# 111116/zdr

Hardware: AMD Instinct MI355X
Metric: Msamples/s fwd+PRB-bwd, cbox 512x512 spp=256 (higher is better)
Workload: dtype f32; 1 GPU; cbox path integrator 512x512 spp=256, forward + PRB backward w.r.t. the 1024x1024x4 material (BASELINE configs[2]); sampler=cmj, accel=brute, rccl_ranks=1, backend=none

## Files before the change

### zdr_amd/csrc/integrators.h

```cpp
#pragma once
#include <type_traits>
#include "accel.h"
#include "internal.h"
#include "microfacet.h"
#include "zdr.h"

ZD float tent_warp1(float u) {
    return (u < 0.5f) ? (fsqrt(2.0f * u) - 1.0f) : (1.0f - fsqrt(2.0f - 2.0f * u));
}

template <int SK, bool PACKED = false>
ZD void pixel_ray(const RenderCfg &R, const SamplerCfg &C, Sampler &smp, int x, int y, f3 &o, f3 &d) {
    f2 off = PACKED ? sampler_pixel_offset<SK>(C, smp) : sampler_next2<SK>(C, smp);
    if (R.use_tent) { off.x = tent_warp1(off.x) + 0.5f; off.y = tent_warp1(off.y) + 0.5f; }
    float px = R.two_over_w * ((float)x + off.x) - 1.0f;
    float py = R.two_over_h * ((float)y + off.y) - 1.0f;
    py *= R.aspect;
    px *= R.cam_tan; py *= R.cam_tan;
    o = ld3(R.cam_o);
    d = normalize((ld3(R.cam_right) * px - ld3(R.cam_upp) * py) + ld3(R.cam_fwd));
}

struct Counters { uint32_t c[8]; };
enum { C_SAMPLES, C_CLOSEST, C_HITS, C_SHADOW, C_SHADED, C_EMIT_BSDF, C_NAN, C_SHADOW_TRACED };
// ... 149 lines not shown
            }
        } else if (ENV && S.env_count > 0) {
            em = env_lookup(S, direction_to_uv(wi));
            pdf_light = env_sampled_light_pdf(S, wi, S.env_count + S.light_count);
            lit = true;
        }
        if (lit && (em.x > 0.0f || em.y > 0.0f || em.z > 0.0f)) {
            GgxTerms g = ggx_terms(wo, wi_local, roughness);
            float pdf_bsdf = ggx_pdf_from(g, wo, wi_local);
            float mis = balanced_heuristic(pdf_bsdf, pdf_light);
            float inv_p = rcp(pdf_bsdf);
            f3 beta = ggx_brdf_from(g, wi_local, diffuse) * inv_p;
            COUNT(C_EMIT_BSDF);
            radiance = radiance + (beta * mis) * em;
            if constexpr (LG) {
                if (h2.slot >= 0) { l_bsdf->w = beta * mis; l_bsdf->light = emit_light_of(S, hit_inst); }
            }
            if (BWD) {
                float dl_; float4 gr = brdf_grad(wi_local.z * ZDR_INV_PI, ggx_dfdr_from(g, wo, wi_local, roughness, dl_), (em * (mis * inv_p)) * le_grad);
                mat_grad.x += gr.x; mat_grad.y += gr.y; mat_grad.z += gr.z; mat_grad.w += gr.w;
            }
        }
        if constexpr (EG) {
            if (h2.slot < 0 && S.env_count > 0) {
                GgxTerms g = ggx_terms(wo, wi_local, roughness);
                float pdf_bsdf = ggx_pdf_from(g, wo, wi_local);
                e_bsdf->w = (ggx_brdf_from(g, wi_local, diffuse) * rcp(pdf_bsdf)) * balanced_heuristic(pdf_bsdf, pdf_light);
                e_bsdf->uv = direction_to_uv(wi);
            }
        }
    }
    if (BWD) { grad = mat_grad; guv = it.uv; }
    return radiance;
}

struct PathVertex {
    f2 uv;
    f3 bW;  float cL, dfLdr;
    f3 neeM;
    f3 bpq; float c, dfdr;
    f3 T, fLW;
    float dlnp;
    int rr;
    f3 bnorm;
};

struct PathState {
    f3 o, d, beta, L;
    float pdf_bsdf;
    int depth;
    Sampler smp;
};

template <bool BWD, bool STATS, bool ENV, bool MT = false>
ZD bool path_arrive(const DScene &S, PathState &ps, const Hit &h, Interaction &it, f3 &term_Li, Counters &cnt, float *term_plfrac = nullptr,
                    const int32_t *inst_slot = nullptr, EnvTerm *env_hit = nullptr, EmitTerm *emit_hit = nullptr) {
    if (h.slot < 0) {
        if (ENV && S.env_count > 0) {
            const f2 euv = direction_to_uv(ps.d);
            f3 em = env_lookup(S, euv);
            float pdf_light = env_sampled_light_pdf(S, ps.d, S.env_count + S.light_count);
            float mis = balanced_heuristic(ps.pdf_bsdf, pdf_light);
            if (env_hit) { env_hit->w = ps.beta * mis; env_hit->uv = euv; }
            ps.L = ps.L + (ps.beta * mis) * em;
            if (BWD) { term_Li = em * mis;
                       if (term_plfrac) *term_plfrac = (ps.pdf_bsdf + pdf_light > 1e-4f) ? pdf_light * rcp(ps.pdf_bsdf + pdf_light) : 0.0f; }
        }
        return true;
    }
    COUNT(C_HITS);
    it = surface_interact(S, h);
    if (dot(-ps.d, it.ng) < 1e-4f || dot(-ps.d, it.ns) < 1e-4f) return true;
    f3 em = xyz(S.emission4[it.inst]);
    if (em.x > 0.0f || em.y > 0.0f || em.z > 0.0f) {
        float pdf_light = sample_light_pdf<ENV>(S, ps.o, it.inst, h.slot, it.p);
        float mis = balanced_heuristic(ps.pdf_bsdf, pdf_light);
        if (emit_hit) { emit_hit->w = ps.beta * mis; emit_hit->light = emit_light_of(S, it.inst); }
        ps.L = ps.L + (ps.beta * mis) * em;
        if (BWD) { term_Li = em * mis;
                   if (term_plfrac) *term_plfrac = (ps.pdf_bsdf + pdf_light > 1e-4f) ? pdf_light * rcp(ps.pdf_bsdf + pdf_light) : 0.0f; }
        if (STATS && ps.depth > 0) cnt.c[C_EMIT_BSDF]++;
        return true;
    }
    if constexpr (MT) {
        it.mat = inst_slot[it.inst];
        return it.mat < 0;
    }
    if (it.inst > 0) return true;
    return false;
}

struct ShadeCtx { f3 diffuse; float roughness; Onb onb; f3 wo, wil; LightSample light; float u_lobe; f2 u_dir; uint32_t i_rr; bool pre; };
struct NeeTerms { f3 dL, bW, fLW, neeM; float cL, dfLdr; };

template <int SK, bool BWD, bool STATS, bool ENV, bool MT = false, bool LG = false>
ZD ShadeCtx shade_ctx(const DScene &S, const RenderCfg &R, const SamplerCfg &C, const KernelIO &io, PathState &ps, const Interaction &it, PathVertex &pv, Counters &cnt,
                      f2 *env_uv = nullptr, int *mesh_light = nullptr) {
    ShadeCtx x;
    float4 m;
    if constexpr (MT) m = read_bsdf_in(io.material, io.mt.m[it.mat], it.uv);
    else m = read_bsdf(io.material, it.uv, R.tex_h, R.tex_w);
    x.diffuse = mk3(m.x, m.y, m.z); x.roughness = m.w;
    COUNT(C_SHADED);
    if (BWD) {
        pv.uv = it.uv; pv.bW = mk3(0.0f); pv.cL = 0.0f; pv.dfLdr = 0.0f; pv.bpq = mk3(0.0f); pv.c = 0.0f; pv.dfdr = 0.0f;
        pv.T = mk3(0.0f); pv.fLW = mk3(0.0f); pv.bnorm = mk3(0.0f); pv.neeM = mk3(0.0f); pv.dlnp = 0.0f; pv.rr = 0;
    }
    x.onb = make_onb(it.ns);
    x.wo = to_local(x.onb, -ps.d);
    x.pre = (SK == 0) && !ENV && cmj_can_batch(C);
    x.u_lobe = 0.0f; x.u_dir.x = 0.0f; x.u_dir.y = 0.0f; x.i_rr = 0u;
    if (x.pre) {
        const VertexSamples v = cmj_vertex_samples(C, ps.smp);
        x.u_lobe = v.u_lobe; x.u_dir = v.u_dir; x.i_rr = v.i_rr;
        x.light = sample_light<ENV, LG>(S, it.p, v.u_pick, [&]() { return v.u_prim; }, [&]() { return v.u_pt; }, env_uv, mesh_light);
    } else {
        float u_pick = sampler_next<SK>(C, ps.smp);
        x.light = sample_light<ENV, LG>(S, it.p, u_pick, [&]() { return sampler_next<SK>(C, ps.smp); }, [&]() { return sampler_next2<SK>(C, ps.smp); }, env_uv, mesh_light);
    }
    x.wil = to_local(x.onb, x.light.wi);
    return x;
}

template <bool BWD, bool EG = false>
ZD NeeTerms nee_terms(const ShadeCtx &x, f3 beta_in, f3 *env_w = nullptr) {
    NeeTerms n; n.dL = n.bW = n.fLW = n.neeM = mk3(0.0f); n.cL = 0.0f; n.dfLdr = 0.0f;
    GgxTerms g = ggx_terms(x.wo, x.wil, x.roughness);
    f3 bsdf = ggx_brdf_from(g, x.wil, x.diffuse);
    float pb = ggx_pdf_from(g, x.wo, x.wil);
    float mis = balanced_heuristic(x.light.pdf, pb);
    float inv_dn = rcp(fmaxf(x.light.pdf, 1e-4f));
    n.dL = (((beta_in * bsdf) * mis) * x.light.eval) * inv_dn;
    if constexpr (EG) *env_w = ((beta_in * bsdf) * mis) * inv_dn;
    if (BWD) {
        f3 W = (x.light.eval * mis) * inv_dn;
        float dlnpL;
        n.bW = beta_in * W; n.cL = x.wil.z * ZDR_INV_PI; n.dfLdr = ggx_dfdr_from(g, x.wo, x.wil, x.roughness, dlnpL);
        n.fLW = bsdf * W;
        float pbf = (x.light.pdf + pb > 1e-4f) ? pb * rcp(x.light.pdf + pb) : 0.0f;
        n.neeM = ((beta_in * bsdf) * W) * (pbf * dlnpL);
    }
    return n;
// ... 136 lines not shown
ZD PrimaryQueue queue_init(const KernelIO &io) {
    PrimaryQueue r; r.base = io.ring + (size_t)blockIdx.x * (ZDR_QUEUE_ENTRIES * 2); r.head = 0; r.tail = 0;
    return r;
}
ZD uint32_t lane_rank(unsigned long long mask) {
    return __builtin_amdgcn_mbcnt_hi((unsigned)(mask >> 32), __builtin_amdgcn_mbcnt_lo((unsigned)mask, 0u));
}

struct NoEnvMiss { ZD void operator()(const EnvTerm &) const {} };
struct NoEmitHit { ZD void operator()(const EmitTerm &) const {} };
template <int SK, class A, bool BWD, bool STATS, bool ENV, bool MT = false, class MISS = NoEnvMiss, class EMIT = NoEmitHit>
ZD void primary_refill(const DScene &S, const RenderCfg &R, const SamplerCfg &C, int *lds, int x, int y, bool valid, unsigned long long cam_mask,
                       uint32_t perm_seed, int bank, uint32_t &next_sample, uint32_t s_end, PrimaryQueue &q, f3 &sum, Counters &cnt,
                       const int32_t *inst_slot = nullptr, MISS on_miss = MISS(), EMIT on_emit = EMIT()) {
    constexpr bool EG = !std::is_same<MISS, NoEnvMiss>::value;
    constexpr bool LG = !std::is_same<EMIT, NoEmitHit>::value;
    for (int b = 0; b < ZDR_RING_BATCH && next_sample < s_end; b++, next_sample++) {
        bool park = false;
        float4 e0 = make_float4(0.0f, 0.0f, 0.0f, 0.0f), e1 = e0;
        EnvTerm miss; env_term_clear(miss);
        if (valid) {
            PathState ps;
            ps.smp = sampler_make<SK>(C, (uint32_t)x, (uint32_t)y, perm_seed, next_sample);
            pixel_ray<SK>(R, C, ps.smp, x, y, ps.o, ps.d);
            ps.beta = mk3(1.0f); ps.L = mk3(0.0f); ps.pdf_bsdf = 1e30f; ps.depth = 0;
            COUNT(C_SAMPLES); COUNT(C_CLOSEST);
            Hit h = A::closest_camera(S, lds, ps.o, ps.d, cam_mask);
            Interaction it; f3 tl;
            EmitTerm seen; emit_term_clear(seen);
            const bool ended = path_arrive<false, STATS, ENV, MT>(S, ps, h, it, tl, cnt, nullptr, inst_slot, EG ? &miss : nullptr, LG ? &seen : nullptr);
            if constexpr (LG) on_emit(seen);
            if (ended) {
                if (!BWD) {
                    if (!any_nan(ps.L)) sum = sum + clamp_radiance(ps.L);
                    else COUNT(C_NAN);
                }
            } else {
                park = true;
                e0 = make_float4(ps.d.x, ps.d.y, ps.d.z, h.u);
                e1 = make_float4(h.v, __int_as_float(h.slot), __uint_as_float(ps.smp.state), __uint_as_float(((uint32_t)threadIdx.x << 26) | ((uint32_t)bank << 25) | next_sample));
            }
        }
        if constexpr (EG) on_miss(miss);
        const unsigned long long m = __ballot(park);
        if (park) {
            float4 *e = q.base + (size_t)((q.tail + lane_rank(m)) % ZDR_QUEUE_ENTRIES) * 2;
            e[0] = e0; e[1] = e1;
        }
        q.tail += (uint32_t)__popcll(m);
    }
    __builtin_amdgcn_fence(__ATOMIC_RELEASE, "wavefront");
}

template <int SK, bool MT = false>
ZD int primary_pop(const DScene &S, const SamplerCfg &C, bool idle, const uint32_t *lds_perm, const int *lds_origin,
                   PrimaryQueue &q, PathState &ps, Interaction &it, const int32_t *inst_slot = nullptr) {
    const unsigned long long m = __ballot(idle);
    const uint32_t avail = q.tail - q.head, rank = lane_rank(m), want = (uint32_t)__popcll(m);
    const bool take = idle && rank < avail;
    int pix = -1;
    __builtin_amdgcn_fence(__ATOMIC_ACQUIRE, "wavefront");
    if (take) {
        const float4 *e = q.base + (size_t)((q.head + rank) % ZDR_QUEUE_ENTRIES) * 2;
        float4 a = e[0], b = e[1];
        Hit h; h.slot = __float_as_int(b.y); h.u = a.w; h.v = b.x; h.t = 0.0f;
        it = surface_interact(S, h);
        if constexpr (MT) it.mat = inst_slot[it.inst];
        ps.d = mk3(a.x, a.y, a.z); ps.o = mk3(0.0f);
        ps.beta = mk3(1.0f); ps.L = mk3(0.0f); ps.pdf_bsdf = 1e30f; ps.depth = 0;
        const uint32_t key = __float_as_uint(b.w);
        const int p = (int)(key >> 26), bank = (int)((key >> 25) & 1u);
        pix = bank * 64 + p;
        ps.smp.px = (uint32_t)(lds_origin[bank * 2] + (p & 7)); ps.smp.py = (uint32_t)(lds_origin[bank * 2 + 1] + (p >> 3));
        ps.smp.sample_index = key & 0x01ffffffu;
        ps.smp.dimension = 2;
        ps.smp.permutation_seed = lds_perm ? lds_perm[pix] : ((SK == 0) ? xxhash32_4(ps.smp.px, ps.smp.py, C.seed, 0u) : 0u);
        ps.smp.state = __float_as_uint(b.z);
    }
    q.head += (want < avail) ? want : avail;
    return pix;
}

struct PackedVertex { float4 a, b, c, d, e; };

ZD PackedVertex pack_vertex(const PathVertex &v, f3 g, int mode = ZDR_PRB_EXPECTATION) {
    PackedVertex p;
    p.a = brdf_grad(v.cL, v.dfLdr, v.bW * g);
    if (mode == ZDR_PRB_EXPECTATION) p.a.w -= dot(g, v.neeM);
    f3 Q = v.bpq * v.c;
    float r = (v.c > 0.0f) ? v.dfdr * rcp(v.c) : 0.0f;
    p.b = make_float4(Q.x, Q.y, Q.z, r);
    p.c = make_float4(v.T.x, v.T.y, v.T.z, v.uv.x);
    f3 gA = g * v.fLW;
    p.d = make_float4(gA.x, gA.y, gA.z, v.uv.y);
    f3 e = (v.rr == 2) ? v.bnorm : ((v.rr == 1) ? mk3(-1.0f, 0.0f, 0.0f) : mk3(0.0f));
    p.e = make_float4(e.x, e.y, e.z, v.dlnp);
    if (mode == ZDR_PRB_DETACHED) p.e = make_float4(0.0f, 0.0f, 0.0f, 0.0f);
    if (mode == ZDR_PRB_LITERAL) p.e = make_float4(v.bnorm.x, v.bnorm.y, v.bnorm.z, 0.0f);
    return p;
}

struct SweepState { f3 A, Lv; float s, Z, tw; };

ZD float4 sweep_vertex(const PackedVertex &p, SweepState &S, f2 &uv, int mode = ZDR_PRB_EXPECTATION) {
    const f3 w = mk3(0.212671f, 0.715160f, 0.072169f);
    f3 Aeff = S.A;
    if (mode == ZDR_PRB_LITERAL) {
        Aeff = mk3(p.e.x, p.e.y, p.e.z) * S.Lv;
    } else if (p.e.x < 0.0f) {
        Aeff = S.A + w * S.s; S.s = 0.0f; S.Z = 0.0f;
    } else if (p.e.x + p.e.y + p.e.z > 0.0f) {
        f3 b = mk3(p.e.x, p.e.y, p.e.z);
        float ba = dot(b, S.A);
        Aeff = S.A - w * ba; S.s += ba; S.Z = dot(b, S.Lv);
    }
    f3 ct = mk3(p.b.x, p.b.y, p.b.z) * Aeff;
    float4 g = make_float4(p.a.x + ct.x, p.a.y + ct.y, p.a.z + ct.z,
                           p.a.w + p.b.w * (ct.x + ct.y + ct.z) + p.e.w * (S.Z + S.tw));
    S.tw = 0.0f;
    f3 T = mk3(p.c.x, p.c.y, p.c.z), gA = mk3(p.d.x, p.d.y, p.d.z);
// ... 6 lines not shown
```

### zdr_amd/csrc/zdr_kernels.hip

```cpp
#include <algorithm>
#include <cstddef>
#include <cstdlib>
#include <map>
#include <mutex>
#include <tuple>
#include <type_traits>
#include "integrators.h"
#include "zdr.h"

#define WAVE 64

struct WorkItem { int x, y, pix; bool valid; uint32_t s_begin, s_end; int chunk, tile, tile_local; };

ZD WorkItem decode_item(const RenderCfg &R, int logical) {
    const int nblocks = R.ntiles * R.nchunks;
    WorkItem w;
    w.valid = logical >= 0 && logical < nblocks;
    const int tl = w.valid ? logical / R.nchunks : 0;
    w.chunk = w.valid ? logical - tl * R.nchunks : 0;
    const int number = tl * R.shard_count + R.shard_index;
    const int ty = number / R.tiles_x;
    int tx = number - ty * R.tiles_x + ty * R.shard_skew;
    tx -= (tx / R.tiles_x) * R.tiles_x;
    w.tile = ty * R.tiles_x + tx; w.tile_local = tl;
// ... 111 lines not shown
struct ItemBanks {
    int logical[2];
    uint32_t inflight[2];
};

struct PathKArgs { DScene S; RenderCfg R; SamplerCfg C; KernelIO io; };
#define ZDR_PATH_KERNEL_PARAMS DScene S_, RenderCfg R_, SamplerCfg C_, KernelIO io_
static constexpr size_t zdr_align_up(size_t x, size_t a) { return (x + a - 1) / a * a; }
static_assert(std::is_trivially_copyable<PathKArgs>::value && std::is_standard_layout<PathKArgs>::value, "kernel arguments are copied bytewise");
static_assert(offsetof(PathKArgs, S) == 0, "first kernel argument at offset 0 of the kernarg segment");
static_assert(offsetof(PathKArgs, R) == zdr_align_up(sizeof(DScene), alignof(RenderCfg)), "PathKArgs does not mirror the kernarg packing");
static_assert(offsetof(PathKArgs, C) == zdr_align_up(offsetof(PathKArgs, R) + sizeof(RenderCfg), alignof(SamplerCfg)), "PathKArgs does not mirror the kernarg packing");
static_assert(offsetof(PathKArgs, io) == zdr_align_up(offsetof(PathKArgs, C) + sizeof(SamplerCfg), alignof(KernelIO)), "PathKArgs does not mirror the kernarg packing");
static_assert(alignof(DScene) <= 8 && alignof(RenderCfg) <= 8 && alignof(SamplerCfg) <= 8 && alignof(KernelIO) <= 8, "an over-aligned member would change the kernarg packing");
typedef __attribute__((address_space(4))) const char karg_byte_t;
ZD const PathKArgs &kargs_fresh() {
    karg_byte_t *p = (karg_byte_t *)__builtin_amdgcn_kernarg_segment_ptr();
    asm volatile("" : "+s"(p));
    return *(const PathKArgs *)p;
}
#define ZDR_KARGS_BEGIN const PathKArgs *ka = &kargs_fresh();
#define ZDR_KARGS_REFRESH ka = &kargs_fresh();
#ifdef ZDR_MEASURE
#define ZDR_ABLATE (R.debug_no_scatter)
#else
#define ZDR_ABLATE 0
#endif

template <int SK, class A, bool STATS, bool ENV, bool MT>
__global__ __launch_bounds__(WAVE, ENV ? A::kMinWavesFwdEnv : A::kMinWavesFwd) void k_path(ZDR_PATH_KERNEL_PARAMS) {
    ZDR_KARGS_BEGIN
#define S (ka->S)
#define R (ka->R)
#define C (ka->C)
#define io (ka->io)
    extern __shared__ int lds[];
    __shared__ uint32_t lds_perm[2 * WAVE];
    __shared__ int lds_origin[4];
    __shared__ float lds_sum[2 * 3 * WAVE];
    const int lane = threadIdx.x;
    Counters cnt;
#pragma unroll
    for (int i = 0; i < 8; i++) cnt.c[i] = 0;
    PathVertex pv; f3 term_Li = mk3(0.0f);
    ItemBanks ib; ib.logical[0] = ib.logical[1] = -1; ib.inflight[0] = ib.inflight[1] = 0;
    int bank = 1;
    bool more_items = true;
    WorkItem w = decode_item(R, -1);
    uint32_t next_sample = 0, s_end = 0, perm_seed = 0;
    unsigned long long cam_mask = 0ull;
    f3 sum = mk3(0.0f);
    PrimaryQueue q = queue_init(io);
    bool alive = false; int pix = 0;
    PathState ps; Interaction it;
    ps.o = mk3(0.0f); ps.d = mk3(0.0f, 0.0f, 1.0f); ps.beta = mk3(1.0f); ps.L = mk3(0.0f); ps.pdf_bsdf = 1e30f; ps.depth = 0;
    ps.smp = sampler_make<SK>(C, 0, 0, 0, 0);
    it.p = mk3(0.0f); it.uv.x = 0.0f; it.uv.y = 0.0f; it.ns = mk3(0.0f, 0.0f, 1.0f); it.ng = it.ns; it.inst = 0; it.prim = 0;
    int stall = 0;
    for (;;) {
        ZDR_KARGS_REFRESH
        bool progress = false;
        if (q.tail - q.head < (uint32_t)__popcll(__ballot(!alive))) {
            if (next_sample < s_end) {
                progress = true;
                const uint32_t t0 = q.tail;
                primary_refill<SK, A, false, STATS, ENV, MT>(S, R, C, lds, w.x, w.y, w.valid, cam_mask, perm_seed, bank, next_sample, s_end, q, sum, cnt,
                                                             MT ? io.mt.inst_slot : nullptr);
                ib.inflight[bank] += q.tail - t0;
            } else if (more_items && ib.logical[bank ^ 1] < 0) {
                if (ib.logical[bank] >= 0) {
                    atomicAdd(&lds_sum[(bank * 3 + 0) * WAVE + lane], sum.x); atomicAdd(&lds_sum[(bank * 3 + 1) * WAVE + lane], sum.y);
                    atomicAdd(&lds_sum[(bank * 3 + 2) * WAVE + lane], sum.z);
                    sum = mk3(0.0f);
                }
                const int nxt = fetch_item(R, io.work_counters);
                if (nxt < 0) more_items = false;
                else {
                    bank ^= 1;
                    ib.logical[bank] = nxt;
                    w = decode_item(R, nxt);
                    perm_seed = (SK == 0) ? xxhash32_4((uint32_t)w.x, (uint32_t)w.y, C.seed, 0u) : 0u;
                    cam_mask = camera_mask(S, io, w);
                    lds_perm[bank * WAVE + lane] = perm_seed;
                    if (lane == 0) { lds_origin[bank * 2] = w.x; lds_origin[bank * 2 + 1] = w.y; }
                    lds_sum[(bank * 3 + 0) * WAVE + lane] = 0.0f; lds_sum[(bank * 3 + 1) * WAVE + lane] = 0.0f; lds_sum[(bank * 3 + 2) * WAVE + lane] = 0.0f;
                    __syncthreads();
                    next_sample = w.s_begin; s_end = w.s_end;
                }
                stall = 0;
                continue;
            }
        }
        const int took = primary_pop<SK, MT>(S, C, !alive, lds_perm, lds_origin, q, ps, it, MT ? io.mt.inst_slot : nullptr);
        if (took >= 0) { alive = true; pix = took; }
        if (__ballot(alive) != 0ull) {
            progress = true;
            bool done = false;
            if (alive) {
                Hit h;
                done = path_shade<SK, A, false, STATS, ENV, MT>(S, R, C, io, lds, ps, it, pv, h, cnt);
                if (!done) { path_continue<A, STATS>(S, lds, ps, h, cnt); done = path_arrive<false, STATS, ENV, MT>(S, ps, h, it, term_Li, cnt, nullptr, MT ? io.mt.inst_slot : nullptr); }
                if (done) {
                    alive = false;
                    if (!any_nan(ps.L)) {
                        f3 c = clamp_radiance(ps.L);
                        const int bk = pix >> 6, px = pix & 63;
                        atomicAdd(&lds_sum[(bk * 3 + 0) * WAVE + px], c.x); atomicAdd(&lds_sum[(bk * 3 + 1) * WAVE + px], c.y);
                        atomicAdd(&lds_sum[(bk * 3 + 2) * WAVE + px], c.z);
                    } else COUNT(C_NAN);
                }
            }
            ib.inflight[0] -= (uint32_t)__popcll(__ballot(done && (pix >> 6) == 0));
            ib.inflight[1] -= (uint32_t)__popcll(__ballot(done && (pix >> 6) == 1));
        }
#pragma unroll
        for (int b = 0; b < 2; b++) {
            if (ib.logical[b] >= 0 && ib.inflight[b] == 0 && (b != bank || next_sample >= s_end)) {
                __syncthreads();
                const WorkItem wb = decode_item(R, ib.logical[b]);
                f3 tot = mk3(lds_sum[(b * 3 + 0) * WAVE + lane], lds_sum[(b * 3 + 1) * WAVE + lane], lds_sum[(b * 3 + 2) * WAVE + lane]);
                if (b == bank) { tot = tot + sum; sum = mk3(0.0f); }
                if (!STATS) store_pixel(R, C, io, wb, tot);
                ib.logical[b] = -1;
            }
        }
        if (__ballot(alive) == 0ull && q.tail == q.head && next_sample >= s_end && !more_items) break;
        stall = progress ? 0 : stall + 1;
        if (stall > 4) { raise_device_error(S, ZDR_DEVERR_STALL); break; }
    }
    flush_counters<STATS>(io, cnt);
#undef S
#undef R
#undef C
#undef io
}

ZD f3 pixel_cotangent(const SamplerCfg &C, const KernelIO &io, int width, uint32_t px, uint32_t py) {
    const float4 gi = io.d_image[px + py * (uint32_t)width];
    f3 g;
    if (C.spp_pow2) g = mk3(gi.x * C.inv_spp, gi.y * C.inv_spp, gi.z * C.inv_spp);
    else { const float fs = (float)C.spp; g = mk3(__fdiv_rn(gi.x, fs), __fdiv_rn(gi.y, fs), __fdiv_rn(gi.z, fs)); }
    if (any_nan(g)) g = mk3(0.0f);
    return g;
}
ZD void env_push(ScatterQueue &q, const KernelIO &io, const RenderCfg &R, f3 g, f2 uv) {
    const float4 g4 = make_float4(g.x, g.y, g.z, 0.0f);
    scatter_push<true, true>(q, io.cells, any_nonzero4(g4) && !any_nan4(g4), uv, g4, R.tex_h, R.tex_w, ZDR_ABLATE, ZDR_ENV_ENTRY, io.mt.m);
}

#define ZDR_EMIT_LDS_LIGHTS 10
ZD void emit_table_init(float *lds_emit) {
    if (threadIdx.x < 3 * ZDR_EMIT_LDS_LIGHTS) lds_emit[threadIdx.x] = 0.0f;
    __builtin_amdgcn_fence(__ATOMIC_RELEASE, "wavefront");
    __builtin_amdgcn_wave_barrier();
// ... 43 lines not shown
    if (S.light_count <= 0) return 0;
    hipLaunchKernelGGL(k_set_emission_values, dim3(S.light_count), dim3(64), 0, st, src, S.light_insts, S.light_range, emission, emission4, light_tris);
    return hipGetLastError() == hipSuccess ? 0 : -1;
}

typedef unsigned int zdr_u4 __attribute__((ext_vector_type(4)));
template <int SK, class A, bool ENV, bool MT, bool EG = false, bool LG = false>
__global__ __launch_bounds__(WAVE, A::kMinWavesBwd) void k_path_bwd(ZDR_PATH_KERNEL_PARAMS) {
    static_assert(!EG || (ENV && MT), "the environment gradient runs in the material-table environment kernels");
    static_assert(!LG || (MT && !EG), "the emission gradient runs in the material-table kernels, without the environment gradient");
    ZDR_KARGS_BEGIN
#define S (ka->S)
#define R (ka->R)
#define C (ka->C)
#define io (ka->io)
    extern __shared__ int lds[];
    __shared__ __attribute__((aligned(16))) float lds_q[ZDR_SCATTER_LDS_FLOATS];
    constexpr int NS = MT ? A::kPoolSlots - 2 : A::kPoolSlots;
    static_assert(NS >= 16 && NS <= 128, "the free mask is two 64-bit words");
    static_assert(ZDR_MAX_MATERIALS <= 256, "a material fits the upper byte of a link");
    typedef typename std::conditional<MT, unsigned short, unsigned char>::type link_t;
    __shared__ float4 lds_pool[5 * NS];
    __shared__ link_t lds_link[NS];
    __shared__ __attribute__((aligned(16))) unsigned int lds_free[4];
    __shared__ int lds_origin[4];
    float *lds_emit = nullptr;
    if constexpr (LG) { __shared__ float lds_emit_table[3 * ZDR_EMIT_LDS_LIGHTS]; lds_emit = lds_emit_table; }
    const int lane = threadIdx.x;
    constexpr unsigned long long all_lo = (NS >= 64) ? ~0ull : ((1ull << (NS & 63)) - 1ull);
    constexpr unsigned long long all_hi = (NS > 64) ? ((NS >= 128) ? ~0ull : ((1ull << ((NS - 64) & 63)) - 1ull)) : 0ull;
    if (lane < 4) {
        const unsigned long long w = (lane < 2) ? all_lo : all_hi;
        lds_free[lane] = (unsigned int)((lane & 1) ? (w >> 32) : w);
    }
    __syncthreads();
    int last = -1;
    int deep_link[ZDR_MAX_RECORDED_DEPTH];
    Counters cnt;
    ItemBanks ib; ib.logical[0] = ib.logical[1] = -1; ib.inflight[0] = ib.inflight[1] = 0;
    int bank = 1;
    bool more_items = true;
    WorkItem w = decode_item(R, -1);
    uint32_t next_sample = 0, s_end = 0, perm_seed = 0;
    unsigned long long cam_mask = 0ull;
    f3 le_grad = mk3(0.0f);
    ScatterQueue q = MT ? scatter_queue_init_cells(lds_q, io.mt.ncells, R.cell_copies) : scatter_queue_init(lds_q, R.tex_h, R.tex_w, R.cell_copies);
    if constexpr (EG) q.lds_cells = nullptr;
    if constexpr (LG) emit_table_init(lds_emit);
    PackedVertex deep[ZDR_MAX_RECORDED_DEPTH];
    int nrec = 0;
    PrimaryQueue pq = queue_init(io);
    f3 unused_sum = mk3(0.0f);
    bool alive = false; int pix = 0;
    PathState ps; Interaction it;
    ps.o = mk3(0.0f); ps.d = mk3(0.0f, 0.0f, 1.0f); ps.beta = mk3(1.0f); ps.L = mk3(0.0f); ps.pdf_bsdf = 1e30f; ps.depth = 0;
    ps.smp = sampler_make<SK>(C, 0, 0, 0, 0);
    it.p = mk3(0.0f); it.uv.x = 0.0f; it.uv.y = 0.0f; it.ns = mk3(0.0f, 0.0f, 1.0f); it.ng = it.ns; it.inst = 0; it.prim = 0;
    int stall = 0;
#ifdef ZDR_MEASURE_STATS
    unsigned long long st_trips = 0, st_shaded = 0, st_fin = 0, st_iters = 0, st_steps = 0;
#endif
    for (;;) {
        ZDR_KARGS_REFRESH
        bool progress = false;
        if (pq.tail - pq.head < (uint32_t)__popcll(__ballot(!alive))) {
            if (next_sample < s_end) {
                const uint32_t t0 = pq.tail;
                if constexpr (EG) {
                    auto camera_miss = [&](const EnvTerm &e) {
                        f3 g = mk3(0.0f);
                        if (w.valid && ((e.w.x != 0.0f) | (e.w.y != 0.0f) | (e.w.z != 0.0f))) g = e.w * pixel_cotangent(C, io, R.width, (uint32_t)w.x, (uint32_t)w.y);
                        env_push(q, io, R, g, e.uv);
                    };
                    primary_refill<SK, A, true, false, ENV, MT>(S, R, C, lds, w.x, w.y, w.valid, cam_mask, perm_seed, bank, next_sample, s_end, pq, unused_sum, cnt,
                                                                io.mt.inst_slot, camera_miss);
                } else if constexpr (LG) {
                    auto camera_emit = [&](const EmitTerm &e) {
                        if (e.light >= 0) emit_add(lds_emit, io, S.light_count, e, pixel_cotangent(C, io, R.width, (uint32_t)w.x, (uint32_t)w.y));
                    };
                    primary_refill<SK, A, true, false, ENV, MT>(S, R, C, lds, w.x, w.y, w.valid, cam_mask, perm_seed, bank, next_sample, s_end, pq, unused_sum, cnt,
                                                                io.mt.inst_slot, NoEnvMiss(), camera_emit);
                } else
                primary_refill<SK, A, true, false, ENV, MT>(S, R, C, lds, w.x, w.y, w.valid, cam_mask, perm_seed, bank, next_sample, s_end, pq, unused_sum, cnt,
                                                            MT ? io.mt.inst_slot : nullptr);
                ib.inflight[bank] += pq.tail - t0;
                progress = true;
            } else if (more_items && ib.logical[bank ^ 1] < 0) {
                const int nxt = fetch_item(R, io.work_counters);
                if (nxt < 0) more_items = false;
                else {
                    bank ^= 1;
                    ib.logical[bank] = nxt;
                    w = decode_item(R, nxt);
                    perm_seed = (SK == 0) ? xxhash32_4((uint32_t)w.x, (uint32_t)w.y, C.seed, 0u) : 0u;
                    cam_mask = camera_mask(S, io, w);
                    if (lane == 0) { lds_origin[bank * 2] = w.x; lds_origin[bank * 2 + 1] = w.y; }
                    __syncthreads();
                    next_sample = w.s_begin; s_end = w.s_end;
                }
                stall = 0;
                continue;
            }
        }
        const int took = primary_pop<SK, MT>(S, C, !alive, nullptr, lds_origin, pq, ps, it, MT ? io.mt.inst_slot : nullptr);
        if (took >= 0) {
            {
                const float4 gi = io.d_image[ps.smp.px + ps.smp.py * (uint32_t)R.width];
                if (C.spp_pow2) le_grad = mk3(gi.x * C.inv_spp, gi.y * C.inv_spp, gi.z * C.inv_spp);
                else { const float fs = (float)C.spp; le_grad = mk3(__fdiv_rn(gi.x, fs), __fdiv_rn(gi.y, fs), __fdiv_rn(gi.z, fs)); }
                if (any_nan(le_grad)) le_grad = mk3(0.0f);
            }
            nrec = 0;
            last = -1;
            alive = true; pix = took;
        }
        if (__ballot(alive) != 0ull) {
            progress = true;
            bool done = false;
            f3 term_Li = mk3(0.0f);
            PackedVertex plast;
            plast.a = plast.b = plast.c = plast.d = plast.e = make_float4(0.0f, 0.0f, 0.0f, 0.0f);
            int pmat = 0;
            int sw_k = -1;
            bool want_store = false, mute = false;
            SweepState sw; sw.A = mk3(0.0f); sw.Lv = mk3(0.0f); sw.s = 0.0f; sw.Z = 0.0f; sw.tw = 0.0f;
            EnvTerm env_nee, env_miss;
            if constexpr (EG) { env_term_clear(env_nee); env_term_clear(env_miss); }
            if (alive) {
                PathVertex pv; float term_plfrac = 0.0f;
                Hit h;
                if (MT) pmat = it.mat;
                if constexpr (EG) done = path_shade<SK, A, true, false, ENV, MT, true>(S, R, C, io, lds, ps, it, pv, h, cnt, &env_nee);
                else if constexpr (LG) {
                    EmitTerm emit_nee;
                    done = path_shade<SK, A, true, false, ENV, MT, false, true>(S, R, C, io, lds, ps, it, pv, h, cnt, nullptr, &emit_nee);
                    emit_add(lds_emit, io, S.light_count, emit_nee, le_grad);
                } else
                done = path_shade<SK, A, true, false, ENV, MT>(S, R, C, io, lds, ps, it, pv, h, cnt);
                plast = pack_vertex(pv, le_grad, R.prb_mode);
                if constexpr (LG) {
                    if (!done) {
                        EmitTerm emit_hit; emit_term_clear(emit_hit);
                        path_continue<A, false>(S, lds, ps, h, cnt);
                        done = path_arrive<true, false, ENV, MT>(S, ps, h, it, term_Li, cnt, &term_plfrac, io.mt.inst_slot, nullptr, &emit_hit);
                        emit_add(lds_emit, io, S.light_count, emit_hit, le_grad);
                    }
                } else
                if constexpr (EG) {
                    if (!done) { path_continue<A, false>(S, lds, ps, h, cnt); done = path_arrive<true, false, ENV, MT>(S, ps, h, it, term_Li, cnt, &term_plfrac, io.mt.inst_slot, &env_miss); }
                } else
                if (!done) { path_continue<A, false>(S, lds, ps, h, cnt); done = path_arrive<true, false, ENV, MT>(S, ps, h, it, term_Li, cnt, &term_plfrac, MT ? io.mt.inst_slot : nullptr); }
                want_store = !done && ZDR_ABLATE != 3;
                nrec++;
                if (done) {
                    alive = false;
                    if (nrec > 0 && ZDR_ABLATE != 3) {
                        mute = any_nan(ps.L);
                        sw_k = nrec - 1;
                        sw.A = le_grad * term_Li; sw.Lv = sw.A; sw.s = 0.0f; sw.Z = 0.0f;
                        sw.tw = (R.prb_mode != ZDR_PRB_EXPECTATION) ? 0.0f : term_plfrac * dot(ps.beta, sw.A);
                    }
                }
            }
            if constexpr (EG) { env_push(q, io, R, env_nee.w * le_grad, env_nee.uv); env_push(q, io, R, env_miss.w * le_grad, env_miss.uv); }
            {
                const unsigned long long req = __ballot(want_store);
                int slot = -1;
                if (req != 0ull) {
                    __builtin_amdgcn_fence(__ATOMIC_ACQUIRE, "wavefront");
                    __builtin_amdgcn_wave_barrier();
                    const zdr_u4 fw = *(volatile const zdr_u4 *)lds_free;
                    unsigned long long free_lo = ((unsigned long long)__builtin_amdgcn_readfirstlane(fw.y) << 32) | (unsigned int)__builtin_amdgcn_readfirstlane(fw.x);
                    unsigned long long free_hi = ((unsigned long long)__builtin_amdgcn_readfirstlane(fw.w) << 32) | (unsigned int)__builtin_amdgcn_readfirstlane(fw.z);
                    const bool home = want_store && lane < NS && ((free_lo >> lane) & 1ull) != 0ull;
                    const unsigned long long took = __ballot(home);
                    free_lo &= ~took;
                    if (home) slot = lane;
                    const unsigned long long rest = req & ~took;
                    if (rest != 0ull && (free_lo | free_hi) != 0ull) {
                        const int nrest = __popcll(rest);
                        const int r = (int)__builtin_amdgcn_mbcnt_hi((unsigned)(rest >> 32), __builtin_amdgcn_mbcnt_lo((unsigned)rest, 0u));
                        const bool mine = want_store && !home;
                        const int cnt_hi = __popcll(free_hi), cnt_lo = __popcll(free_lo);
                        const bool fh = ((free_hi >> lane) & 1ull) != 0ull;
                        const int jh = (int)__builtin_amdgcn_mbcnt_hi((unsigned)(free_hi >> 32), __builtin_amdgcn_mbcnt_lo((unsigned)free_hi, 0u));
                        const int at_hi = __builtin_amdgcn_ds_permute((fh ? jh : cnt_hi + (lane - jh)) << 2, lane);
                        const int pick_hi = __builtin_amdgcn_ds_bpermute(r << 2, at_hi);
                        if (mine && r < cnt_hi) slot = 64 + pick_hi;
                        free_hi &= ~__ballot(fh && jh < nrest);
                        const int r2 = r - cnt_hi, nrest2 = nrest - cnt_hi;
                        const bool fl = ((free_lo >> lane) & 1ull) != 0ull;
                        const int jl = (int)__builtin_amdgcn_mbcnt_hi((unsigned)(free_lo >> 32), __builtin_amdgcn_mbcnt_lo((unsigned)free_lo, 0u));
                        const int at_lo = __builtin_amdgcn_ds_permute((fl ? jl : cnt_lo + (lane - jl)) << 2, lane);
                        const int pick_lo = __builtin_amdgcn_ds_bpermute((r2 & 63) << 2, at_lo);
                        if (mine && r2 >= 0 && r2 < cnt_lo) slot = pick_lo;
                        free_lo &= ~__ballot(fl && jl < nrest2);
                    }
                    if (lane == 0) {
                        const zdr_u4 nw = {(unsigned int)free_lo, (unsigned int)(free_lo >> 32), (unsigned int)free_hi, (unsigned int)(free_hi >> 32)};
                        *(volatile zdr_u4 *)lds_free = nw;
                    }
                    __builtin_amdgcn_fence(__ATOMIC_RELEASE, "wavefront");
                    __builtin_amdgcn_wave_barrier();
                }
                if (want_store) {
                    if (slot >= 0) {
                        float4 *r = lds_pool + slot;
                        r[0] = plast.a; r[NS] = plast.b; r[2 * NS] = plast.c; r[3 * NS] = plast.d; r[4 * NS] = plast.e;
                        lds_link[slot] = MT ? (link_t)((last & 255) | (pmat << 8)) : (link_t)last;
                        last = slot;
                    } else {
                        deep[nrec - 1] = plast; deep_link[nrec - 1] = MT ? ((last & 255) | (pmat << 8)) : last;
                        last = 255;
                    }
                }
            }
            ib.inflight[0] -= (uint32_t)__popcll(__ballot(done && (pix >> 6) == 0));
            ib.inflight[1] -= (uint32_t)__popcll(__ballot(done && (pix >> 6) == 1));
            PackedVertex cur = plast;
            int cur_mat = pmat;
            int loc = last;
#ifdef ZDR_MEASURE_STATS
            st_trips++; st_shaded += (unsigned long long)__popcll(__ballot(alive || done));
            st_fin += (unsigned long long)__popcll(__ballot(sw_k >= 0));
#endif
            int sweep_cap = (ZDR_ABLATE == 4) ? 2 : ((ZDR_ABLATE == 5) ? 1 : 64);
            while (__ballot(sw_k >= 0) != 0ull && sweep_cap-- > 0) {
                const bool swp = sw_k >= 0;
#ifdef ZDR_MEASURE_STATS
                st_iters++; st_steps += (unsigned long long)__popcll(__ballot(swp));
#endif
                float4 g = make_float4(0.0f, 0.0f, 0.0f, 0.0f);
                f2 guv; guv.x = 0.0f; guv.y = 0.0f;
                const int gmat = cur_mat;
                if (swp) { g = sweep_vertex(cur, sw, guv, R.prb_mode); sw_k--; }
                asm volatile("" : "+v"(g.x), "+v"(g.y), "+v"(g.z), "+v"(g.w), "+v"(guv.x), "+v"(guv.y), "+v"(sw.A.x), "+v"(sw.A.y), "+v"(sw.A.z),
                             "+v"(sw.Lv.x), "+v"(sw.Lv.y), "+v"(sw.Lv.z), "+v"(sw.s), "+v"(sw.Z), "+v"(sw.tw) : : "memory");
                const bool fetch = swp && sw_k >= 0;
                const bool pooled = fetch && loc != 255;
                int nloc = -1;
                if (pooled) {
                    const float4 *r = lds_pool + loc;
                    cur.a = r[0]; cur.b = r[NS]; cur.c = r[2 * NS]; cur.d = r[3 * NS]; cur.e = r[4 * NS];
                    nloc = (int)lds_link[loc];
                    if (MT) { cur_mat = nloc >> 8; nloc &= 255; }
                }
                asm volatile("" ::: "memory");
                if (fetch && loc == 255) {
                    cur = deep[sw_k]; nloc = deep_link[sw_k];
                    if (MT) { cur_mat = nloc >> 8; nloc &= 255; }
                }
                if (pooled) __hip_atomic_fetch_or(&lds_free[loc >> 5], 1u << (loc & 31), __ATOMIC_RELEASE, __HIP_MEMORY_SCOPE_WAVEFRONT);
                if (fetch) loc = nloc;
                scatter_push<MT, EG>(q, io.cells, swp && !mute && any_nonzero4(g) && !any_nan4(g), guv, g, R.tex_h, R.tex_w, ZDR_ABLATE, gmat, io.mt.m);
            }
        }
#pragma unroll
        for (int b = 0; b < 2; b++)
            if (ib.logical[b] >= 0 && ib.inflight[b] == 0 && (b != bank || next_sample >= s_end)) ib.logical[b] = -1;
        if (__ballot(alive) == 0ull && pq.tail == pq.head && next_sample >= s_end && !more_items) break;
        stall = progress ? 0 : stall + 1;
        if (stall > 4) { raise_device_error(S, ZDR_DEVERR_STALL); break; }
    }
    scatter_finish<MT, EG>(q, io.cells, R.tex_h, R.tex_w, ZDR_ABLATE, io.mt.m);
    if constexpr (LG) emit_table_finish(lds_emit, io, S.light_count);
    {
        __builtin_amdgcn_fence(__ATOMIC_ACQUIRE, "wavefront");
        __builtin_amdgcn_wave_barrier();
        const zdr_u4 fw = *(volatile const zdr_u4 *)lds_free;
        const bool whole = fw.x == (unsigned int)all_lo && fw.y == (unsigned int)(all_lo >> 32) && fw.z == (unsigned int)all_hi && fw.w == (unsigned int)(all_hi >> 32);
        if (!whole && lane == 0 && stall <= 4 && ZDR_ABLATE == 0) raise_device_error(S, ZDR_DEVERR_POOL);
    }
#ifdef ZDR_MEASURE_STATS
    if (lane == 0) {
        atomicAdd(io.counters + 0, st_trips); atomicAdd(io.counters + 1, st_shaded); atomicAdd(io.counters + 2, st_fin);
        atomicAdd(io.counters + 3, st_iters); atomicAdd(io.counters + 4, st_steps);
        atomicAdd(io.counters + 5, q.st_flushes); atomicAdd(io.counters + 6, q.st_entries); atomicAdd(io.counters + 7, q.st_dups);
    }
#endif
#undef S
#undef R
#undef C
#undef io
}

template <int INTEG, int SK, class A, bool BWD, bool STATS, bool ENV, bool MT, bool EG = false, bool LG = false>
#ifndef ZDR_MIN_WAVES_DIRECT
#define ZDR_MIN_WAVES_DIRECT 4
#endif
__global__ __launch_bounds__(WAVE, (INTEG == ZDR_DIRECT && !A::kNeedsLds) ? (ENV ? 3 : ZDR_MIN_WAVES_DIRECT) : 1) void k_simple(ZDR_PATH_KERNEL_PARAMS) {
    static_assert(!LG || (INTEG == ZDR_DIRECT && BWD && !STATS && MT && !EG), "the emission gradient runs in the direct backward material-table kernels, without the environment gradient");
    ZDR_KARGS_BEGIN
#define S (ka->S)
#define R (ka->R)
#define C (ka->C)
#define io (ka->io)
    extern __shared__ int lds[];
    __shared__ __attribute__((aligned(16))) float lds_q[BWD ? ZDR_SCATTER_LDS_FLOATS : 4];
    float *lds_emit = nullptr;
    if constexpr (LG) { __shared__ float lds_emit_table[3 * ZDR_EMIT_LDS_LIGHTS]; lds_emit = lds_emit_table; }
    const WorkItem w = decode_block(R);
    const uint32_t perm_seed = (SK == 0) ? xxhash32_4((uint32_t)w.x, (uint32_t)w.y, C.seed, 0u) : 0u;
    Counters cnt;
#pragma unroll
    for (int i = 0; i < 8; i++) cnt.c[i] = 0;
    f3 le_grad = mk3(0.0f);
    if (BWD) le_grad = load_le_grad(C, io, w);
    ScatterQueue q = MT ? scatter_queue_init_cells(lds_q, io.mt.ncells, R.cell_copies) : scatter_queue_init(lds_q, R.tex_h, R.tex_w, R.cell_copies);
    if constexpr (EG) q.lds_cells = nullptr;
    if constexpr (LG) emit_table_init(lds_emit);
    const unsigned long long cam_mask = camera_mask(S, io, w);
    f3 sum = mk3(0.0f);
// ... 480 lines not shown
```

Baseline: 7581 Msamples/s.

## Carry compact Hit across wavefront loop iterations instead of full Interaction

The persistent-wave forward and PRB backward loops now carry only the compact Hit record across iterations and rebuild the surface Interaction at the start of each shading step. Arrival checks such as emission and back-facing tests are deferred to the next iteration. In backward, a path that terminates late pops its already-stored vertex before the sweep. This is meant to cut live registers across the loop and unify the primary-pop and continuation paths, at the cost of an extra loop trip for terminating paths and more control flow in the sweep setup. An asm barrier on the bank-reset store is also added to steer codegen.

Result: no change. 7624 Msamples/s (median of 6 runs) (+0.6%).

```diff
diff --git a/zdr_amd/csrc/integrators.h b/zdr_amd/csrc/integrators.h
--- a/zdr_amd/csrc/integrators.h
+++ b/zdr_amd/csrc/integrators.h
@@ -225,24 +225,22 @@
     Sampler smp;
 };
 
-template <bool BWD, bool STATS, bool ENV, bool MT = false>
-ZD bool path_arrive(const DScene &S, PathState &ps, const Hit &h, Interaction &it, f3 &term_Li, Counters &cnt, float *term_plfrac = nullptr,
-                    const int32_t *inst_slot = nullptr, EnvTerm *env_hit = nullptr, EmitTerm *emit_hit = nullptr) {
-    if (h.slot < 0) {
-        if (ENV && S.env_count > 0) {
-            const f2 euv = direction_to_uv(ps.d);
-            f3 em = env_lookup(S, euv);
-            float pdf_light = env_sampled_light_pdf(S, ps.d, S.env_count + S.light_count);
-            float mis = balanced_heuristic(ps.pdf_bsdf, pdf_light);
-            if (env_hit) { env_hit->w = ps.beta * mis; env_hit->uv = euv; }
-            ps.L = ps.L + (ps.beta * mis) * em;
-            if (BWD) { term_Li = em * mis;
-                       if (term_plfrac) *term_plfrac = (ps.pdf_bsdf + pdf_light > 1e-4f) ? pdf_light * rcp(ps.pdf_bsdf + pdf_light) : 0.0f; }
-        }
-        return true;
-    }
-    COUNT(C_HITS);
-    it = surface_interact(S, h);
+template <bool BWD, bool ENV>
+ZD void path_arrive_miss(const DScene &S, PathState &ps, f3 &term_Li, float *term_plfrac = nullptr, EnvTerm *env_hit = nullptr) {
+    if (ENV && S.env_count > 0) {
+        const f2 euv = direction_to_uv(ps.d);
+        f3 em = env_lookup(S, euv);
+        float pdf_light = env_sampled_light_pdf(S, ps.d, S.env_count + S.light_count);
+        float mis = balanced_heuristic(ps.pdf_bsdf, pdf_light);
+        if (env_hit) { env_hit->w = ps.beta * mis; env_hit->uv = euv; }
+        ps.L = ps.L + (ps.beta * mis) * em;
+        if (BWD) { term_Li = em * mis;
+                   if (term_plfrac) *term_plfrac = (ps.pdf_bsdf + pdf_light > 1e-4f) ? pdf_light * rcp(ps.pdf_bsdf + pdf_light) : 0.0f; }
+    }
+}
+template <bool BWD, bool STATS, bool ENV, bool MT = false, bool HAVE_MAT = false>
+ZD bool path_arrive_checks(const DScene &S, PathState &ps, const Hit &h, Interaction &it, f3 &term_Li, Counters &cnt, float *term_plfrac = nullptr,
+                           const int32_t *inst_slot = nullptr, EmitTerm *emit_hit = nullptr) {
     if (dot(-ps.d, it.ng) < 1e-4f || dot(-ps.d, it.ns) < 1e-4f) return true;
     f3 em = xyz(S.emission4[it.inst]);
     if (em.x > 0.0f || em.y > 0.0f || em.z > 0.0f) {
@@ -256,11 +254,19 @@
         return true;
     }
     if constexpr (MT) {
-        it.mat = inst_slot[it.inst];
+        if (!HAVE_MAT) it.mat = inst_slot[it.inst];
         return it.mat < 0;
     }
     if (it.inst > 0) return true;
     return false;
+}
+template <bool BWD, bool STATS, bool ENV, bool MT = false>
+ZD bool path_arrive(const DScene &S, PathState &ps, const Hit &h, Interaction &it, f3 &term_Li, Counters &cnt, float *term_plfrac = nullptr,
+                    const int32_t *inst_slot = nullptr, EnvTerm *env_hit = nullptr, EmitTerm *emit_hit = nullptr) {
+    if (h.slot < 0) { path_arrive_miss<BWD, ENV>(S, ps, term_Li, term_plfrac, env_hit); return true; }
+    COUNT(C_HITS);
+    it = surface_interact(S, h);
+    return path_arrive_checks<BWD, STATS, ENV, MT>(S, ps, h, it, term_Li, cnt, term_plfrac, inst_slot, emit_hit);
 }
 
 struct ShadeCtx { f3 diffuse; float roughness; Onb onb; f3 wo, wil; LightSample light; float u_lobe; f2 u_dir; uint32_t i_rr; bool pre; };
@@ -503,9 +509,8 @@
     __builtin_amdgcn_fence(__ATOMIC_RELEASE, "wavefront");
 }
 
-template <int SK, bool MT = false>
-ZD int primary_pop(const DScene &S, const SamplerCfg &C, bool idle, const uint32_t *lds_perm, const int *lds_origin,
-                   PrimaryQueue &q, PathState &ps, Interaction &it, const int32_t *inst_slot = nullptr) {
+template <int SK>
+ZD int primary_pop(const SamplerCfg &C, bool idle, const uint32_t *lds_perm, const int *lds_origin, PrimaryQueue &q, PathState &ps, Hit &h) {
     const unsigned long long m = __ballot(idle);
     const uint32_t avail = q.tail - q.head, rank = lane_rank(m), want = (uint32_t)__popcll(m);
     const bool take = idle && rank < avail;
@@ -514,9 +519,7 @@
     if (take) {
         const float4 *e = q.base + (size_t)((q.head + rank) % ZDR_QUEUE_ENTRIES) * 2;
         float4 a = e[0], b = e[1];
-        Hit h; h.slot = __float_as_int(b.y); h.u = a.w; h.v = b.x; h.t = 0.0f;
-        it = surface_interact(S, h);
-        if constexpr (MT) it.mat = inst_slot[it.inst];
+        h.slot = __float_as_int(b.y); h.u = a.w; h.v = b.x; h.t = 0.0f;
         ps.d = mk3(a.x, a.y, a.z); ps.o = mk3(0.0f);
         ps.beta = mk3(1.0f); ps.L = mk3(0.0f); ps.pdf_bsdf = 1e30f; ps.depth = 0;
         const uint32_t key = __float_as_uint(b.w);
diff --git a/zdr_amd/csrc/zdr_kernels.hip b/zdr_amd/csrc/zdr_kernels.hip
--- a/zdr_amd/csrc/zdr_kernels.hip
+++ b/zdr_amd/csrc/zdr_kernels.hip
@@ -187,10 +187,11 @@
     f3 sum = mk3(0.0f);
     PrimaryQueue q = queue_init(io);
     bool alive = false; int pix = 0;
-    PathState ps; Interaction it;
+    PathState ps;
+    Hit hh;
     ps.o = mk3(0.0f); ps.d = mk3(0.0f, 0.0f, 1.0f); ps.beta = mk3(1.0f); ps.L = mk3(0.0f); ps.pdf_bsdf = 1e30f; ps.depth = 0;
     ps.smp = sampler_make<SK>(C, 0, 0, 0, 0);
-    it.p = mk3(0.0f); it.uv.x = 0.0f; it.uv.y = 0.0f; it.ns = mk3(0.0f, 0.0f, 1.0f); it.ng = it.ns; it.inst = 0; it.prim = 0;
+    hh.slot = 0; hh.u = 0.0f; hh.v = 0.0f; hh.t = 0.0f;
     int stall = 0;
     for (;;) {
         ZDR_KARGS_REFRESH
@@ -226,15 +227,26 @@
                 continue;
             }
         }
-        const int took = primary_pop<SK, MT>(S, C, !alive, lds_perm, lds_origin, q, ps, it, MT ? io.mt.inst_slot : nullptr);
+        const bool arriving = alive;
+        const int took = primary_pop<SK>(C, !alive, lds_perm, lds_origin, q, ps, hh);
         if (took >= 0) { alive = true; pix = took; }
         if (__ballot(alive) != 0ull) {
             progress = true;
             bool done = false;
             if (alive) {
-                Hit h;
-                done = path_shade<SK, A, false, STATS, ENV, MT>(S, R, C, io, lds, ps, it, pv, h, cnt);
-                if (!done) { path_continue<A, STATS>(S, lds, ps, h, cnt); done = path_arrive<false, STATS, ENV, MT>(S, ps, h, it, term_Li, cnt, nullptr, MT ? io.mt.inst_slot : nullptr); }
+                Interaction it = surface_interact(S, hh);
+                if constexpr (MT) it.mat = io.mt.inst_slot[it.inst];
+                if (arriving) {
+                    COUNT(C_HITS);
+                    done = path_arrive_checks<false, STATS, ENV, MT, true>(S, ps, hh, it, term_Li, cnt);
+                }
+                if (!done) {
+                    done = path_shade<SK, A, false, STATS, ENV, MT>(S, R, C, io, lds, ps, it, pv, hh, cnt);
+                    if (!done) {
+                        path_continue<A, STATS>(S, lds, ps, hh, cnt);
+                        if (hh.slot < 0) { path_arrive_miss<false, ENV>(S, ps, term_Li); done = true; }
+                    }
+                }
                 if (done) {
                     alive = false;
                     if (!any_nan(ps.L)) {
@@ -384,10 +396,11 @@
     PrimaryQueue pq = queue_init(io);
     f3 unused_sum = mk3(0.0f);
     bool alive = false; int pix = 0;
-    PathState ps; Interaction it;
+    PathState ps;
+    Hit hh;
     ps.o = mk3(0.0f); ps.d = mk3(0.0f, 0.0f, 1.0f); ps.beta = mk3(1.0f); ps.L = mk3(0.0f); ps.pdf_bsdf = 1e30f; ps.depth = 0;
     ps.smp = sampler_make<SK>(C, 0, 0, 0, 0);
-    it.p = mk3(0.0f); it.uv.x = 0.0f; it.uv.y = 0.0f; it.ns = mk3(0.0f, 0.0f, 1.0f); it.ng = it.ns; it.inst = 0; it.prim = 0;
+    hh.slot = 0; hh.u = 0.0f; hh.v = 0.0f; hh.t = 0.0f;
     int stall = 0;
 #ifdef ZDR_MEASURE_STATS
     unsigned long long st_trips = 0, st_shaded = 0, st_fin = 0, st_iters = 0, st_steps = 0;
@@ -434,7 +447,8 @@
                 continue;
             }
         }
-        const int took = primary_pop<SK, MT>(S, C, !alive, nullptr, lds_origin, pq, ps, it, MT ? io.mt.inst_slot : nullptr);
+        const bool arriving = alive;
+        const int took = primary_pop<SK>(C, !alive, nullptr, lds_origin, pq, ps, hh);
         if (took >= 0) {
             {
                 const float4 gi = io.d_image[ps.smp.px + ps.smp.py * (uint32_t)R.width];
@@ -449,6 +463,7 @@
         if (__ballot(alive) != 0ull) {
             progress = true;
             bool done = false;
+            bool late = false;
             f3 term_Li = mk3(0.0f);
             PackedVertex plast;
             plast.a = plast.b = plast.c = plast.d = plast.e = make_float4(0.0f, 0.0f, 0.0f, 0.0f);
@@ -460,37 +475,42 @@
             if constexpr (EG) { env_term_clear(env_nee); env_term_clear(env_miss); }
             if (alive) {
                 PathVertex pv; float term_plfrac = 0.0f;
-                Hit h;
-                if (MT) pmat = it.mat;
-                if constexpr (EG) done = path_shade<SK, A, true, false, ENV, MT, true>(S, R, C, io, lds, ps, it, pv, h, cnt, &env_nee);
-                else if constexpr (LG) {
-                    EmitTerm emit_nee;
-                    done = path_shade<SK, A, true, false, ENV, MT, false, true>(S, R, C, io, lds, ps, it, pv, h, cnt, nullptr, &emit_nee);
-                    emit_add(lds_emit, io, S.light_count, emit_nee, le_grad);
-                } else
-                done = path_shade<SK, A, true, false, ENV, MT>(S, R, C, io, lds, ps, it, pv, h, cnt);
-                plast = pack_vertex(pv, le_grad, R.prb_mode);
-                if constexpr (LG) {
+                Interaction it = surface_interact(S, hh);
+                if constexpr (MT) it.mat = io.mt.inst_slot[it.inst];
+                if (arriving) {
+                    f3 tl = mk3(0.0f); float tp = 0.0f;
+                    if constexpr (LG) {
+                        EmitTerm emit_hit; emit_term_clear(emit_hit);
+                        late = path_arrive_checks<true, false, ENV, MT, true>(S, ps, hh, it, tl, cnt, &tp, nullptr, &emit_hit);
+                        emit_add(lds_emit, io, S.light_count, emit_hit, le_grad);
+                    } else late = path_arrive_checks<true, false, ENV, MT, true>(S, ps, hh, it, tl, cnt, &tp);
+                    if (late) { ps.o = le_grad * tl; ps.pdf_bsdf = tp * dot(ps.beta, ps.o); }
+                }
+                if (!late) {
+                    if (MT) pmat = it.mat;
+                    if constexpr (EG) done = path_shade<SK, A, true, false, ENV, MT, true>(S, R, C, io, lds, ps, it, pv, hh, cnt, &env_nee);
+                    else if constexpr (LG) {
+                        EmitTerm emit_nee;
+                        done = path_shade<SK, A, true, false, ENV, MT, false, true>(S, R, C, io, lds, ps, it, pv, hh, cnt, nullptr, &emit_nee);
+                        emit_add(lds_emit, io, S.light_count, emit_nee, le_grad);
+                    } else
+                    done = path_shade<SK, A, true, false, ENV, MT>(S, R, C, io, lds, ps, it, pv, hh, cnt);
+                    plast = pack_vertex(pv, le_grad, R.prb_mode);
                     if (!done) {
-                        EmitTerm emit_hit; emit_term_clear(emit_hit);
-                        path_continue<A, false>(S, lds, ps, h, cnt);
-                        done = path_arrive<true, false, ENV, MT>(S, ps, h, it, term_Li, cnt, &term_plfrac, io.mt.inst_slot, nullptr, &emit_hit);
-                        emit_add(lds_emit, io, S.light_count, emit_hit, le_grad);
+                        path_continue<A, false>(S, lds, ps, hh, cnt);
+                        if (hh.slot < 0) { path_arrive_miss<true, ENV>(S, ps, term_Li, &term_plfrac, EG ? &env_miss : nullptr); done = true; }
                     }
-                } else
-                if constexpr (EG) {
-                    if (!done) { path_continue<A, false>(S, lds, ps, h, cnt); done = path_arrive<true, false, ENV, MT>(S, ps, h, it, term_Li, cnt, &term_plfrac, io.mt.inst_slot, &env_miss); }
-                } else
-                if (!done) { path_continue<A, false>(S, lds, ps, h, cnt); done = path_arrive<true, false, ENV, MT>(S, ps, h, it, term_Li, cnt, &term_plfrac, MT ? io.mt.inst_slot : nullptr); }
-                want_store = !done && ZDR_ABLATE != 3;
-                nrec++;
+                    want_store = !done && ZDR_ABLATE != 3;
+                    nrec++;
+                } else done = true;
                 if (done) {
                     alive = false;
                     if (nrec > 0 && ZDR_ABLATE != 3) {
                         mute = any_nan(ps.L);
                         sw_k = nrec - 1;
-                        sw.A = le_grad * term_Li; sw.Lv = sw.A; sw.s = 0.0f; sw.Z = 0.0f;
-                        sw.tw = (R.prb_mode != ZDR_PRB_EXPECTATION) ? 0.0f : term_plfrac * dot(ps.beta, sw.A);
+                        sw.A = late ? ps.o : le_grad * term_Li; sw.Lv = sw.A; sw.s = 0.0f; sw.Z = 0.0f;
+                        const float tw = late ? ps.pdf_bsdf : term_plfrac * dot(ps.beta, sw.A);
+                        sw.tw = (R.prb_mode != ZDR_PRB_EXPECTATION) ? 0.0f : tw;
                     }
                 }
             }
@@ -552,8 +572,19 @@
             PackedVertex cur = plast;
             int cur_mat = pmat;
             int loc = last;
+            if (late && sw_k >= 0) {
+                int nloc;
+                if (loc != 255) {
+                    const float4 *r = lds_pool + loc;
+                    cur.a = r[0]; cur.b = r[NS]; cur.c = r[2 * NS]; cur.d = r[3 * NS]; cur.e = r[4 * NS];
+                    nloc = (int)lds_link[loc];
+                    __hip_atomic_fetch_or(&lds_free[loc >> 5], 1u << (loc & 31), __ATOMIC_RELEASE, __HIP_MEMORY_SCOPE_WAVEFRONT);
+                } else { cur = deep[sw_k]; nloc = deep_link[sw_k]; }
+                if (MT) { cur_mat = nloc >> 8; nloc &= 255; }
+                loc = nloc;
+            }
 #ifdef ZDR_MEASURE_STATS
-            st_trips++; st_shaded += (unsigned long long)__popcll(__ballot(alive || done));
+            st_trips++; st_shaded += (unsigned long long)__popcll(__ballot((alive || done) && !late));
             st_fin += (unsigned long long)__popcll(__ballot(sw_k >= 0));
 #endif
             int sweep_cap = (ZDR_ABLATE == 4) ? 2 : ((ZDR_ABLATE == 5) ? 1 : 64);
@@ -589,7 +620,11 @@
         }
 #pragma unroll
         for (int b = 0; b < 2; b++)
-            if (ib.logical[b] >= 0 && ib.inflight[b] == 0 && (b != bank || next_sample >= s_end)) ib.logical[b] = -1;
+            if (ib.logical[b] >= 0 && ib.inflight[b] == 0 && (b != bank || next_sample >= s_end)) {
+                int none = -1;
+                asm volatile("" : "+v"(none));
+                ib.logical[b] = none;
+            }
         if (__ballot(alive) == 0ull && pq.tail == pq.head && next_sample >= s_end && !more_items) break;
         stall = progress ? 0 : stall + 1;
         if (stall > 4) { raise_device_error(S, ZDR_DEVERR_STALL); break; }
```
